# Shuijing725/CrowdNav_Prediction_AttnGraph

Hardware: NVIDIA H100
Metric: env_steps_per_s_ppo_rollout (higher is better)
Workload: dtype f32

## Files before the change

### crowdnav_prediction_attngraph_b200/csrc/cn_gemm_tc.cu

```cuda
#include "cn_gemm_tc.h"

__global__ void cn_split_f16_kernel(const float* __restrict__ src, float scale, __half* __restrict__ hi,
                                    __half* __restrict__ lo, size_t count) {
  const size_t i = (size_t)blockIdx.x * blockDim.x + threadIdx.x;
  if (i >= count) return;
  const float x = fminf(fmaxf(src[i] * scale, -65504.0f), 65504.0f);
  const __half h = __float2half_rn(x);
  hi[i] = h;
  lo[i] = __float2half_rn(x - __half2float(h));
}

namespace {

typedef CUresult (*EncodeFn)(CUtensorMap*, CUtensorMapDataType, cuuint32_t, void*, const cuuint64_t*, const cuuint64_t*,
                             const cuuint32_t*, const cuuint32_t*, CUtensorMapInterleave, CUtensorMapSwizzle,
                             CUtensorMapL2promotion, CUtensorMapFloatOOBfill);

EncodeFn get_encode() {
  static EncodeFn fn = nullptr;
  if (!fn) {
    void* sym = nullptr;
    cudaDriverEntryPointQueryResult qres;
    if (cudaGetDriverEntryPoint("cuTensorMapEncodeTiled", &sym, cudaEnableDefault, &qres) == cudaSuccess &&
        qres == cudaDriverEntryPointSuccess)
// ... 4 lines not shown

int halloc16(CnLaunchCtx* c, __half** ptr, size_t count) {
  float* q = nullptr;
  int rc = palloc(c, &q, (count + 1) / 2);
  *ptr = reinterpret_cast<__half*>(q);
  return rc;
}

int tc_store_maps(TcMat& t, int rows, int K) {
  if (!tma_store_ok(t.hi, (size_t)t.pitch * 2) || !tma_store_ok(t.lo, (size_t)t.pitch * 2)) return 0;
  int rc = make_store_map(&t.sh, t.hi, 2, rows, K, t.pitch);
  if (!rc) rc = make_store_map(&t.sl, t.lo, 2, rows, K, t.pitch);
  return rc;
}

typedef void (*TcKernel)(CUtensorMap, CUtensorMap, CUtensorMap, CUtensorMap, int, int, int, TcEpilogue, CUtensorMap,
                         CUtensorMap, CUtensorMap);
template <int BN>
TcKernel tc_kernel(int act, int out) {
  static const TcKernel k[3][3] = {
      {cn_gemm_tc_kernel<BN, false, CN_ACT_NONE, TC_OUT_F32>, cn_gemm_tc_kernel<BN, false, CN_ACT_NONE, TC_OUT_F16>,
       cn_gemm_tc_kernel<BN, false, CN_ACT_NONE, TC_OUT_BOTH>},
      {cn_gemm_tc_kernel<BN, false, CN_ACT_RELU, TC_OUT_F32>, cn_gemm_tc_kernel<BN, false, CN_ACT_RELU, TC_OUT_F16>,
       cn_gemm_tc_kernel<BN, false, CN_ACT_RELU, TC_OUT_BOTH>},
      {cn_gemm_tc_kernel<BN, false, CN_ACT_TANH, TC_OUT_F32>, cn_gemm_tc_kernel<BN, false, CN_ACT_TANH, TC_OUT_F16>,
       cn_gemm_tc_kernel<BN, false, CN_ACT_TANH, TC_OUT_BOTH>}};
  return k[act][out - 1];
}

#ifdef CN_GEMM_TRACE
unsigned long long* g_tc_trace = nullptr;
int g_tc_trace_cap = 0;
// ... 28 lines not shown
  CUresult r = enc(&s->map, esize == 4 ? CU_TENSOR_MAP_DATA_TYPE_FLOAT32 : CU_TENSOR_MAP_DATA_TYPE_FLOAT16, 2,
                   const_cast<void*>(ptr), gdim, gstride, box, estr, CU_TENSOR_MAP_INTERLEAVE_NONE,
                   CU_TENSOR_MAP_SWIZZLE_128B, CU_TENSOR_MAP_L2_PROMOTION_NONE, CU_TENSOR_MAP_FLOAT_OOB_FILL_NONE);
  if (r != CUDA_SUCCESS) return cn_set_error("cuTensorMapEncodeTiled(store) failed (%d) rows=%d cols=%d", (int)r, rows, cols);
  s->rows = rows; s->cols = cols;
  return 0;
}

int tc_alloc(CnLaunchCtx* c, TcMat& t, int rows, int K, int box_rows, int box_k) {
  int rc = halloc16(c, &t.hi, (size_t)rows * K);
  if (!rc) rc = halloc16(c, &t.lo, (size_t)rows * K);
  t.pitch = K; t.box_k = box_k;
  if (!rc) rc = make_map(&t.mh, t.hi, rows, K, box_rows, K, box_k);
  if (!rc) rc = make_map(&t.ml, t.lo, rows, K, box_rows, K, box_k);
  if (!rc) rc = tc_store_maps(t, rows, K);
  return rc;
}

int tc_view(TcMat& v, const TcMat& src, int col0, int rows, int K, int box_rows) {
  v.hi = src.hi + col0; v.lo = src.lo + col0; v.pitch = src.pitch; v.box_k = src.box_k;
  int rc = make_map(&v.mh, v.hi, rows, K, box_rows, src.pitch, src.box_k);
  if (!rc) rc = make_map(&v.ml, v.lo, rows, K, box_rows, src.pitch, src.box_k);
  if (!rc) rc = tc_store_maps(v, rows, K);
  return rc;
}

void split16(CnLaunchCtx* c, cudaStream_t st, const float* src, float scale, __half* hi, __half* lo, size_t count) {
  cn_split_f16_kernel<<<(unsigned)((count + 255) / 256), 256, 0, st>>>(src, scale, hi, lo, count);
  c->launches += 1;
}
// ... 5 lines not shown
      if (e == cudaSuccess)
        e = cudaFuncSetAttribute(tc_kernel<256>(act, out), cudaFuncAttributeMaxDynamicSharedMemorySize, TcCfg<256>::kSmemBytes);
      if (e == cudaSuccess)
        e = cudaFuncSetAttribute(tc_kernel<64>(act, out), cudaFuncAttributeMaxDynamicSharedMemorySize, TcCfg<64>::kSmemBytes);
    }
  if (e == cudaSuccess)
    e = cudaFuncSetAttribute(cn_gemm_tc_kernel<64, true>, cudaFuncAttributeMaxDynamicSharedMemorySize, TcCfg<64>::kSmemBytes);
  if (e == cudaSuccess)
    e = cudaFuncSetAttribute(cn_gemm_tc_kernel<256, false, CN_ACT_NONE, TC_OUT_GRU>,
                             cudaFuncAttributeMaxDynamicSharedMemorySize, TcCfg<256>::kSmemBytes);
  if (e != cudaSuccess) return cn_set_error("cudaFuncSetAttribute(tc): %s", cudaGetErrorString(e));
  return 0;
}

void gemm_tc(CnLaunchCtx* c, cudaStream_t st, const TcMat& A, const TcMat& B, int M, int N, int K, int bn, const float* bias,
             int act, const TcOut& o, const int* m_ptr, int act_lo, int act_hi, const int* m0_ptr) {
  TcEpilogue ep;
  memset(&ep, 0, sizeof(ep));
  ep.bias = bias; ep.inv_scale = 1.0f / 64.0f; ep.act = act; ep.act_lo = act_lo; ep.act_hi = act_hi;
  ep.c32 = o.c32; ep.ldc = o.ldc; ep.out_hi = o.oh; ep.out_lo = o.ol; ep.ldh = o.ldh; ep.m_ptr = m_ptr; ep.m0_ptr = m0_ptr;
  {
    static const int nostore = (getenv("CN_DBG_NOSTORE") && getenv("CN_DBG_NOSTORE")[0] == '1') ? 1 : 0;
    ep.dbg_nostore = nostore;
  }
  if (A.box_k != tc_box_k(bn) || B.box_k != tc_box_k(bn)) {
    if (!c->launch_error) {
      c->launch_error = true;
      cn_set_error("gemm_tc in stage '%s': operand boxes %d / %d wide, the BN = %d instance loads %d",
                   c->cur_stage ? c->cur_stage : "?", A.box_k, B.box_k, bn, tc_box_k(bn));
    }
    return;
  }
  const int out_kind = (o.c32 ? TC_OUT_F32 : 0) | (o.oh ? TC_OUT_F16 : 0);
  if (act < CN_ACT_NONE || act > CN_ACT_TANH || !out_kind) {
    if (!c->launch_error) {
      c->launch_error = true;
      cn_set_error("gemm_tc in stage '%s': activation %d / no output", c->cur_stage ? c->cur_stage : "?", act);
    }
    return;
  }
#ifdef CN_GEMM_TRACE
  ep.trace = g_tc_trace; ep.trace_cap = g_tc_trace_cap;
#endif
  static const CUtensorMap no_map = {};
// ... 3 lines not shown
    const bool ok = (!o.c32 || fits(o.sc)) && (!o.oh || (fits(o.sh) && fits(o.sl)));
    if (!ok) {
      if (!c->launch_error) {
        c->launch_error = true;
        cn_set_error("gemm_tc in stage '%s': a BN = 256 output needs a TMA store map of [%d x %d] (16-byte-aligned "
                     "base, row pitch a multiple of 16 bytes)", c->cur_stage ? c->cur_stage : "?", M, N);
      }
      return;
    }
    if (o.c32) mc = &o.sc->map;
    if (o.oh) { mh = &o.sh->map; ml = &o.sl->map; }
  }
  const int tiles = (N / bn) * ((M + TC_BM - 1) / TC_BM);
  dim3 grid(tiles < c->num_sms ? tiles : c->num_sms);
  if (bn == 256)
    launch_k(c, tc_kernel<256>(act, out_kind), grid, dim3(TC_THREADS), TcCfg<256>::kSmemBytes, st, A.mh, A.ml, B.mh, B.ml, M, N, K, ep,
             *mc, *mh, *ml);
  else
    launch_k(c, tc_kernel<64>(act, out_kind), grid, dim3(TC_THREADS), TcCfg<64>::kSmemBytes, st, A.mh, A.ml, B.mh, B.ml, M, N, K, ep,
             *mc, *mh, *ml);
}

void gemm_tc_gru(CnLaunchCtx* c, cudaStream_t st, const TcMat& A, const TcMat& B, int M, const float* bias,
                 const float* h_in, const float* mask, float* h_out, int group, int pitch, int off, __half* oh, __half* ol,
                 int ldh) {
  const int N = 4 * 256, K = 64 + 256;
  if (A.box_k != tc_box_k(256) || B.box_k != tc_box_k(256) || !bias || !h_out || !mask || group <= 0) {
    if (!c->launch_error) {
      c->launch_error = true;
      cn_set_error("gemm_tc_gru in stage '%s': operand boxes %d / %d wide (need %d), or a missing bias / mask / output",
                   c->cur_stage ? c->cur_stage : "?", A.box_k, B.box_k, tc_box_k(256));
    }
    return;
  }
  TcEpilogue ep;
  memset(&ep, 0, sizeof(ep));
  ep.bias = bias; ep.inv_scale = 1.0f / 64.0f; ep.act_hi = 1 << 30;
  ep.c32 = h_out; ep.ldc = 256; ep.out_hi = oh; ep.out_lo = ol; ep.ldh = ldh;
  ep.gru_h = h_in; ep.gru_mask = mask; ep.gru_group = group; ep.gru_pitch = pitch; ep.gru_off = off;
  static const CUtensorMap no_map = {};
  const int tiles = (N / 256) * ((M + TC_BM - 1) / TC_BM);
  dim3 grid(tiles < c->num_sms ? tiles : c->num_sms);
  launch_k(c, cn_gemm_tc_kernel<256, false, CN_ACT_NONE, TC_OUT_GRU>, grid, dim3(TC_THREADS), TcCfg<256>::kSmemBytes, st,
           A.mh, A.ml, B.mh, B.ml, M, N, K, ep, no_map, no_map, no_map);
}

int gemm_tc_promote(int num_sms, cudaStream_t st, const __half* ahi, const __half* alo, int a_rows, int a_pitch,
                    const __half* bhi, const __half* blo, int b_rows, int b_pitch, int Kd, float* C, int ldc,
                    const float* bias, int act, const float* inv_a, const float* inv_b, int ksplit) {
  const int bn = 64;
  if (b_rows % bn) return cn_set_error("cn_update gemm: output columns %d not a multiple of 64", b_rows);
  const int Kp = (Kd + TC_BK - 1) / TC_BK * TC_BK;
  CUtensorMap mah, mal, mbh, mbl;
  int rc = make_map(&mah, ahi, a_rows, Kd, TC_BM, a_pitch);
  if (!rc) rc = make_map(&mal, alo, a_rows, Kd, TC_BM, a_pitch);
  if (!rc) rc = make_map(&mbh, bhi, b_rows, Kd, bn, b_pitch);
  if (!rc) rc = make_map(&mbl, blo, b_rows, Kd, bn, b_pitch);
  if (rc) return rc;
  TcEpilogue ep;
  memset(&ep, 0, sizeof(ep));
  ep.bias = bias; ep.inv_scale = 1.0f; ep.act = act; ep.act_lo = 0; ep.act_hi = 1 << 30;
  ep.c32 = C; ep.ldc = ldc; ep.inv_scale_a = inv_a; ep.inv_scale_b = inv_b; ep.ksplit = ksplit;
  const int tiles = (b_rows / bn) * ((a_rows + TC_BM - 1) / TC_BM) * (ksplit > 1 ? ksplit : 1);
  const int grid = tiles < num_sms ? tiles : num_sms;
  static const CUtensorMap no_map = {};
  cn_gemm_tc_kernel<64, true><<<grid, TC_THREADS, TcCfg<64>::kSmemBytes, st>>>(mah, mal, mbh, mbl, a_rows, b_rows, Kp, ep,
                                                                                no_map, no_map, no_map);
  cudaError_t e = cudaGetLastError();
  if (e != cudaSuccess) return cn_set_error("cn_update gemm launch (M=%d N=%d K=%d ksplit=%d): %s", a_rows, b_rows, Kd, ksplit, cudaGetErrorString(e));
  return 0;
}

extern "C" {

int cn_internal_gemm_tc_ex(const float* dA, const float* dW, const float* dbias, float* dC, int M, int N, int K, int act,
                           int bn, const int* m_ptr, const int* m0_ptr, int a_col0, int a_pitch, __half* out_hi,
                           __half* out_lo, int ldh, int act_lo, int act_hi) {
  if (a_pitch == 0) a_pitch = K;
  if ((bn != 256 && bn != 64) || M <= 0 || N <= 0 || K <= 0 || N % bn || K % TC_BK || a_col0 < 0 ||
      a_col0 + K > a_pitch || a_col0 % 8 || a_pitch % 8 || (!dC && !out_hi) || (!out_hi != !out_lo) ||
      (out_hi && ldh < N))
    return cn_set_error("cn_internal_gemm_tc_ex: need bn in {64,256}, M, N, K > 0, N %% bn == 0, K %% 64 == 0, "
                        "a_col0 + K <= a_pitch (both multiples of 8), an output and ldh >= N");
  if (bn == 256 && ((dC && !tma_store_ok(dC, (size_t)N * 4)) ||
                    (out_hi && (!tma_store_ok(out_hi, (size_t)ldh * 2) || !tma_store_ok(out_lo, (size_t)ldh * 2)))))
    return cn_set_error("cn_internal_gemm_tc_ex: a BN = 256 output needs a 16-byte-aligned base and a row pitch that is "
                        "a multiple of 16 bytes");
  CnLaunchCtx ctx;
  cudaDeviceGetAttribute(&ctx.num_sms, cudaDevAttrMultiProcessorCount, 0);
  TcMat Af, A, B;
  int rc = tc_alloc(&ctx, Af, M, a_pitch, TC_BM, tc_box_k(bn));
  if (!rc) rc = tc_view(A, Af, a_col0, M, K, TC_BM);
  if (!rc) rc = tc_alloc(&ctx, B, N, K, bn, tc_box_k(bn));
  if (!rc) rc = tc_set_attrs();
  TcOut o = out32(dC, N);
  o.oh = out_hi; o.ol = out_lo; o.ldh = ldh;
  TcStoreMap sc, sh, sl;
  if (bn == 256) {
    if (!rc && dC) rc = make_store_map(&sc, dC, 4, M, N, N);
    if (!rc && out_hi) rc = make_store_map(&sh, out_hi, 2, M, N, ldh);
    if (!rc && out_hi) rc = make_store_map(&sl, out_lo, 2, M, N, ldh);
    o.sc = &sc; o.sh = &sh; o.sl = &sl;
  }
  if (!rc) {
    split16(&ctx, 0, dA, 1.0f, Af.hi, Af.lo, (size_t)M * a_pitch);
    split16(&ctx, 0, dW, 64.0f, B.hi, B.lo, (size_t)N * K);
    gemm_tc(&ctx, 0, A, B, M, N, K, bn, dbias, act, o, m_ptr, act_lo, act_hi > 0 ? act_hi : 1 << 30, m0_ptr);
    cudaError_t err = cudaDeviceSynchronize();
    if (err != cudaSuccess) rc = cn_set_error("cn_internal_gemm_tc_ex: %s", cudaGetErrorString(err));
    else if (ctx.launch_error) rc = 1;
  }
  cn_launch_free(&ctx);
  return rc;
}
int cn_internal_gemm_tc(const float* dA, const float* dW, const float* dbias, float* dC, int M, int N, int K, int act,
                        int bn) {
  return cn_internal_gemm_tc_ex(dA, dW, dbias, dC, M, N, K, act, bn, nullptr, nullptr, 0, 0, nullptr, nullptr, 0, 0, 0);
}

#ifdef CN_GEMM_TRACE
int cn_internal_gemm_trace(unsigned long long* dtrace, int cap) {
  g_tc_trace = dtrace; g_tc_trace_cap = dtrace ? cap : 0;
  return 0;
}
#endif

}
```

### crowdnav_prediction_attngraph_b200/csrc/cn_gemm_tc.cuh

```cuda
#pragma once
#include <cuda.h>
#include <cuda_fp16.h>
#include <cuda_runtime.h>
#include <stdint.h>

#include "cn_launch.cuh"

#define TC_BM 128
#define TC_BK 64
#define TC_CONSUMER_WARPS 8
#define TC_THREADS (128 + 32 * TC_CONSUMER_WARPS)

template <int BN>
struct TcCfg {
  static constexpr int kBK = (BN >= 256) ? 32 : TC_BK;
  static constexpr int kSwizzle = 2 * kBK;
  static constexpr int kStages = 4;
  static constexpr int kATile = TC_BM * kBK * 2;
  static constexpr int kBTile = BN * kBK * 2;
  static constexpr int kStageBytes = 2 * kATile + 2 * kBTile;
  static constexpr int kStoreBoxes = (BN >= 256) ? 2 : 0;
  static constexpr int kBoxBytes = 64 * 128;
  static constexpr int kStagingBytes = 2 * kStoreBoxes * kBoxBytes;
  static constexpr int kSmemBytes = kStages * kStageBytes + kStagingBytes + 256  + 1024 ;
};

struct TcEpilogue {
  const float* bias;
  float inv_scale;
  int act;
  int act_lo, act_hi;
  float* c32;
  int ldc;
  __half* out_hi;
  __half* out_lo;
  int ldh;
  const int* m_ptr;
  int dbg_nostore;
  const int* m0_ptr;
  const float* inv_scale_a;
  const float* inv_scale_b;
  int ksplit;
  const float* gru_h;
  const float* gru_mask;
  int gru_group, gru_pitch, gru_off;
#ifdef CN_GEMM_TRACE
  unsigned long long* trace;
  int trace_cap;
#endif
};

#ifdef CN_GEMM_TRACE
#define TC_TRACE_REC 7
#define TC_TRACE_WAIT_CLK 100
#endif

enum { TC_OUT_F32 = 1, TC_OUT_F16 = 2, TC_OUT_BOTH = 3, TC_OUT_GRU = 4 };

#ifdef CN_GEMM_TRACE
#define TC_TRACE(...) __VA_ARGS__
#else
#define TC_TRACE(...)
#endif

namespace tc {

__device__ __forceinline__ uint32_t smem_u32(const void* p) { return (uint32_t)__cvta_generic_to_shared(p); }

// ... 82 lines not shown

template <int N>
__device__ __forceinline__ void wgmma_f16(float (&d)[N / 2], uint64_t da, uint64_t db, uint32_t accum);
template <>
__device__ __forceinline__ void wgmma_f16<64>(float (&d)[32], uint64_t da, uint64_t db, uint32_t accum) {
  asm volatile(
      "{\n.reg .pred p;\nsetp.ne.b32 p, %34, 0;\n"
      "wgmma.mma_async.sync.aligned.m64n64k16.f32.f16.f16 {"
      "%0, %1, %2, %3, %4, %5, %6, %7, %8, %9, %10, %11, %12, %13, %14, %15, "
      "%16, %17, %18, %19, %20, %21, %22, %23, %24, %25, %26, %27, %28, %29, %30, %31"
      "}, %32, %33, p, 1, 1, 0, 0;\n}\n"
      : "+f"(d[0]), "+f"(d[1]), "+f"(d[2]), "+f"(d[3]), "+f"(d[4]), "+f"(d[5]), "+f"(d[6]), "+f"(d[7]),
        "+f"(d[8]), "+f"(d[9]), "+f"(d[10]), "+f"(d[11]), "+f"(d[12]), "+f"(d[13]), "+f"(d[14]), "+f"(d[15]),
        "+f"(d[16]), "+f"(d[17]), "+f"(d[18]), "+f"(d[19]), "+f"(d[20]), "+f"(d[21]), "+f"(d[22]), "+f"(d[23]),
        "+f"(d[24]), "+f"(d[25]), "+f"(d[26]), "+f"(d[27]), "+f"(d[28]), "+f"(d[29]), "+f"(d[30]), "+f"(d[31])
      : "l"(da), "l"(db), "r"(accum));
}
template <>
__device__ __forceinline__ void wgmma_f16<192>(float (&d)[96], uint64_t da, uint64_t db, uint32_t accum) {
  asm volatile(
      "{\n.reg .pred p;\nsetp.ne.b32 p, %98, 0;\n"
      "wgmma.mma_async.sync.aligned.m64n192k16.f32.f16.f16 {"
      "%0, %1, %2, %3, %4, %5, %6, %7, %8, %9, %10, %11, %12, %13, %14, %15, "
      "%16, %17, %18, %19, %20, %21, %22, %23, %24, %25, %26, %27, %28, %29, %30, %31, "
      "%32, %33, %34, %35, %36, %37, %38, %39, %40, %41, %42, %43, %44, %45, %46, %47, "
      "%48, %49, %50, %51, %52, %53, %54, %55, %56, %57, %58, %59, %60, %61, %62, %63, "
      "%64, %65, %66, %67, %68, %69, %70, %71, %72, %73, %74, %75, %76, %77, %78, %79, "
      "%80, %81, %82, %83, %84, %85, %86, %87, %88, %89, %90, %91, %92, %93, %94, %95"
      "}, %96, %97, p, 1, 1, 0, 0;\n}\n"
      : "+f"(d[0]), "+f"(d[1]), "+f"(d[2]), "+f"(d[3]), "+f"(d[4]), "+f"(d[5]), "+f"(d[6]), "+f"(d[7]),
// ... 114 lines not shown
#else
      tc::bulk_wait_read<PENDING>();
#endif
    }
    tc::named_bar_sync(bar_id, 128);
  }
  __device__ __forceinline__ void release() {
    tc::fence_proxy_async_smem();
    tc::named_bar_sync(bar_id, 128);
  }
  __device__ __forceinline__ uint32_t buf(uint32_t b) const { return base + (b % TcCfg<256>::kStoreBoxes) * TcCfg<256>::kBoxBytes; }
};

template <int ACT, int OUT>
__device__ __forceinline__ void tc_epilogue_tma(const float (&acc)[128], const TcEpilogue& ep, float inv_scale, int n0,
                                                int m_half, int wr, int lane, TcStaging& sg, const CUtensorMap* map_c,
                                                const CUtensorMap* map_oh, const CUtensorMap* map_ol) {
  static_assert(ACT >= 0 && ACT <= 2 && OUT >= TC_OUT_F32 && OUT <= TC_OUT_BOTH, "epilogue kind");
  constexpr int NB = TcCfg<256>::kStoreBoxes;
  static_assert(NB >= 2 && (NB & (NB - 1)) == 0, "the split fp16 output stages hi and lo boxes together");
  const int cq = 2 * (lane & 3);
  const bool issue = sg.leader && !ep.dbg_nostore;
  const uint32_t rsw = (uint32_t)(wr & 7);
  const uint32_t row_off = (uint32_t)wr * 128u;
  if constexpr ((OUT & TC_OUT_F32) != 0) {
#pragma unroll
    for (int j = 0; j < 8; ++j) {
      sg.acquire<NB - 1>();
      const uint32_t b = sg.buf(sg.box) + row_off + 8u * (uint32_t)(lane & 1);
#pragma unroll
      for (int q = 0; q < 4; ++q) {
        const int g = 4 * j + q, col = n0 + 8 * g + cq;
        const float b0 = ep.bias ? __ldg(ep.bias + col) : 0.0f, b1 = ep.bias ? __ldg(ep.bias + col + 1) : 0.0f;
        const bool w0 = col >= ep.act_lo && col < ep.act_hi, w1 = col + 1 >= ep.act_lo && col + 1 < ep.act_hi;
        const uint32_t chunk = (uint32_t)(2 * q + ((lane & 3) >> 1));
#pragma unroll
        for (int h = 0; h < 2; ++h) {
          float v0 = fmaf(acc[4 * g + 2 * h], inv_scale, b0), v1 = fmaf(acc[4 * g + 2 * h + 1], inv_scale, b1);
          if constexpr (ACT == 1) {
            v0 = w0 ? fmaxf(v0, 0.0f) : v0; v1 = w1 ? fmaxf(v1, 0.0f) : v1;
          } else if constexpr (ACT == 2) {
            if (w0) v0 = tc::fast_tanh(v0);
// ... 1 lines not shown
          }
          tc::st_shared_v2(b + 1024u * h + ((chunk ^ rsw) << 4), v0, v1);
        }
      }
      sg.release();
      if (issue) {
        tc::tma_store_2d(map_c, sg.buf(sg.box), n0 + 32 * j, m_half);
        tc::bulk_commit();
      }
      ++sg.box;
    }
  }
  if constexpr ((OUT & TC_OUT_F16) != 0) {
#pragma unroll
    for (int j = 0; j < 4; ++j) {
      sg.acquire<NB - 2>();
      const uint32_t bh = sg.buf(sg.box) + row_off + 4u * (uint32_t)(lane & 3);
      const uint32_t bl = sg.buf(sg.box + 1) + row_off + 4u * (uint32_t)(lane & 3);
#pragma unroll
      for (int q = 0; q < 8; ++q) {
        const int g = 8 * j + q, col = n0 + 8 * g + cq;
        const float b0 = ep.bias ? __ldg(ep.bias + col) : 0.0f, b1 = ep.bias ? __ldg(ep.bias + col + 1) : 0.0f;
        const bool w0 = col >= ep.act_lo && col < ep.act_hi, w1 = col + 1 >= ep.act_lo && col + 1 < ep.act_hi;
        const uint32_t sw_off = ((uint32_t)q ^ rsw) << 4;
#pragma unroll
        for (int h = 0; h < 2; ++h) {
          float v0 = fmaf(acc[4 * g + 2 * h], inv_scale, b0), v1 = fmaf(acc[4 * g + 2 * h + 1], inv_scale, b1);
          if constexpr (ACT == 1) {
            v0 = w0 ? fmaxf(v0, 0.0f) : v0; v1 = w1 ? fmaxf(v1, 0.0f) : v1;
          } else if constexpr (ACT == 2) {
// ... 49 lines not shown
        o[k] = (1.0f - z) * n + z * hv[k];
      }
      if (ep.dbg_nostore) continue;
      *reinterpret_cast<float2*>(ep.c32 + orow * 256 + u) = make_float2(o[0], o[1]);
      if (ep.out_hi) {
        uint32_t lo;
        const uint32_t hi = tc::split_pair_hi(o[0], o[1], &lo);
        const size_t q = (size_t)row * ep.ldh + u;
        *reinterpret_cast<uint32_t*>(ep.out_hi + q) = hi;
        *reinterpret_cast<uint32_t*>(ep.out_lo + q) = lo;
      }
    }
  }
}

template <int BN, bool PROMOTE = false, int ACT = 0, int OUT = TC_OUT_F32>
__global__ void __launch_bounds__(TC_THREADS, 1)
cn_gemm_tc_kernel(const __grid_constant__ CUtensorMap map_ahi, const __grid_constant__ CUtensorMap map_alo,
                  const __grid_constant__ CUtensorMap map_bhi, const __grid_constant__ CUtensorMap map_blo,
                  int M, int N, int K, TcEpilogue ep, const __grid_constant__ CUtensorMap map_c,
                  const __grid_constant__ CUtensorMap map_oh, const __grid_constant__ CUtensorMap map_ol) {
  cn_pdl_trigger();
  constexpr int TC_STAGES = TcCfg<BN>::kStages;
  constexpr int BK = TcCfg<BN>::kBK;
  constexpr int SW = TcCfg<BN>::kSwizzle;
  constexpr int TC_A_TILE_BYTES = TcCfg<BN>::kATile;
  constexpr int TC_B_TILE_BYTES = TcCfg<BN>::kBTile;
  constexpr int TC_STAGE_BYTES = TcCfg<BN>::kStageBytes;
  constexpr bool kTmaStore = !PROMOTE && BN == 256 && OUT != TC_OUT_GRU;
  static_assert(OUT != TC_OUT_GRU || (BN == 256 && !PROMOTE), "the GRU epilogue reads four 64-column gate blocks");
  static_assert(!PROMOTE || BK == 64, "PROMOTE sums 64-wide k-blocks");
  static_assert(!kTmaStore || TcCfg<BN>::kStoreBoxes > 0, "BN = 256 stages its output");
  extern __shared__ uint8_t tc_smem_raw[];
  const uint32_t raw = tc::smem_u32(tc_smem_raw);
  const uint32_t base = (raw + 1023u) & ~1023u;
  const uint32_t staging = base + TC_STAGES * TC_STAGE_BYTES;
  const uint32_t bar_base = staging + TcCfg<BN>::kStagingBytes;
  const uint32_t bar_full = bar_base, bar_empty = bar_base + 64;

  const int warp = threadIdx.x >> 5, lane = threadIdx.x & 31, wg = warp >> 2;
  const int num_kb = K / BK;

  if (threadIdx.x == 0) {
    for (int s = 0; s < TC_STAGES; ++s) {
      tc::mbar_init(bar_full + 8 * s, 1);
      tc::mbar_init(bar_empty + 8 * s, TC_CONSUMER_WARPS);
    }
    asm volatile("fence.mbarrier_init.release.cluster;" ::: "memory");
    asm volatile("prefetch.tensormap [%0];" ::"l"(&map_ahi) : "memory");
    asm volatile("prefetch.tensormap [%0];" ::"l"(&map_alo) : "memory");
    asm volatile("prefetch.tensormap [%0];" ::"l"(&map_bhi) : "memory");
    asm volatile("prefetch.tensormap [%0];" ::"l"(&map_blo) : "memory");
    if constexpr (kTmaStore) {
      if constexpr ((OUT & TC_OUT_F32) != 0) asm volatile("prefetch.tensormap [%0];" ::"l"(&map_c) : "memory");
      if constexpr ((OUT & TC_OUT_F16) != 0) {
        asm volatile("prefetch.tensormap [%0];" ::"l"(&map_oh) : "memory");
        asm volatile("prefetch.tensormap [%0];" ::"l"(&map_ol) : "memory");
      }
    }
  }
  __syncthreads();
  cn_pdl_wait();
  const int m_ext = M;
  if (ep.m_ptr) { const int mc = *ep.m_ptr; M = mc < M ? mc : M; }
  int m_lo = ep.m0_ptr ? *ep.m0_ptr : 0;
  if (m_lo > M) m_lo = M;
  const int n_ntiles = N / BN;
  const int n_mn = ((M - m_lo + TC_BM - 1) / TC_BM) * n_ntiles;
  const int ksplit = (PROMOTE && ep.ksplit > 1) ? ep.ksplit : 1;
  const int kb_per = (num_kb + ksplit - 1) / ksplit;
  const int n_tiles = n_mn * ksplit;

  if (wg == 0) {
    tc::setmaxnreg_dec<40>();
    if (threadIdx.x == 0) {
      uint32_t it = 0;
      for (int tile = blockIdx.x; tile < n_tiles; tile += gridDim.x) {
        const int mn = tile % n_mn, ks = tile / n_mn;
        const int m0 = m_lo + (mn / n_ntiles) * TC_BM, n0 = (mn % n_ntiles) * BN;
        const int kb0 = ks * kb_per, kb1 = (kb0 + kb_per < num_kb) ? kb0 + kb_per : num_kb;
        for (int kb = kb0; kb < kb1; ++kb, ++it) {
          const uint32_t s = it % TC_STAGES, ph = (it / TC_STAGES) & 1u;
          tc::mbar_wait(bar_empty + 8 * s, ph ^ 1u);
          const uint32_t full = bar_full + 8 * s;
          tc::mbar_expect_tx(full, TC_STAGE_BYTES);
          const uint32_t st = base + s * TC_STAGE_BYTES;
          tc::tma_load_2d(st, &map_ahi, full, kb * BK, m0);
          tc::tma_load_2d(st + TC_A_TILE_BYTES, &map_alo, full, kb * BK, m0);
          tc::tma_load_2d(st + 2 * TC_A_TILE_BYTES, &map_bhi, full, kb * BK, n0);
          tc::tma_load_2d(st + 2 * TC_A_TILE_BYTES + TC_B_TILE_BYTES, &map_blo, full, kb * BK, n0);
        }
      }
    }
    return;
  }
  tc::setmaxnreg_inc<232>();
  float inv_scale = ep.inv_scale;
  if (ep.inv_scale_a) inv_scale *= __ldg(ep.inv_scale_a);
  if (ep.inv_scale_b) inv_scale *= __ldg(ep.inv_scale_b);
  const int half = wg - 1;
  const int wr = 16 * (warp & 3) + (lane >> 2);
  const int cq = 2 * (lane & 3);
  uint32_t it = 0;
  TcStaging sg;
  sg.base = staging + half * TcCfg<BN>::kStoreBoxes * TcCfg<BN>::kBoxBytes;
  sg.box = 0; sg.leader = (threadIdx.x & 127) == 0; sg.bar_id = wg;
  TC_TRACE(sg.waits = 0; sg.wait_clk = 0;)
  TC_TRACE(const bool tr = ep.trace && warp == 4 && lane == 0; int tr_n = 0;)
  for (int tile = blockIdx.x; tile < n_tiles; tile += gridDim.x) {
    const int mn = tile % n_mn, ks = tile / n_mn;
    const int m0 = m_lo + (mn / n_ntiles) * TC_BM, n0 = (mn % n_ntiles) * BN;
    const int kb0 = ks * kb_per, kb1 = (kb0 + kb_per < num_kb) ? kb0 + kb_per : num_kb;
    TC_TRACE(const uint64_t t_tile = tc::globaltimer(); uint64_t t_first = 0; uint32_t polls = 0;)
    float acc[BN / 2];
    float sum[PROMOTE ? BN / 2 : 1];
    if constexpr (PROMOTE) {
#pragma unroll
      for (int i = 0; i < BN / 2; ++i) sum[i] = 0.0f;
    }
    uint32_t prev = 0;
    for (int kb = kb0; kb < kb1; ++kb, ++it) {
      const uint32_t s = it % TC_STAGES, ph = (it / TC_STAGES) & 1u;
#ifdef CN_GEMM_TRACE
      polls += tc::mbar_wait_polls(bar_full + 8 * s, ph);
      if (kb == kb0) t_first = tc::globaltimer();
#else
      tc::mbar_wait(bar_full + 8 * s, ph);
#endif
      const uint32_t st = base + s * TC_STAGE_BYTES;
      const uint32_t a_hi = st + half * (TC_A_TILE_BYTES / 2), a_lo = a_hi + TC_A_TILE_BYTES,
                     b_hi = st + 2 * TC_A_TILE_BYTES, b_lo = b_hi + TC_B_TILE_BYTES;
      tc::fence_regs(acc);
      tc::wgmma_fence();
#pragma unroll
      for (int k = 0; k < BK / 16; ++k) {
        const uint32_t koff = k * 32;
        const uint64_t dah = tc::make_desc<SW>(a_hi + koff), dal = tc::make_desc<SW>(a_lo + koff);
        const uint64_t dbh = tc::make_desc<SW>(b_hi + koff), dbl = tc::make_desc<SW>(b_lo + koff);
        const bool first = k == 0 && (PROMOTE || kb == kb0);
        tc::wgmma_f16<BN>(acc, dah, dbh, first ? 0u : 1u);
        tc::wgmma_f16<BN>(acc, dah, dbl, 1u);
        tc::wgmma_f16<BN>(acc, dal, dbh, 1u);
      }
      tc::wgmma_commit();
      tc::fence_regs(acc);
      if constexpr (PROMOTE) {
        tc::wgmma_wait<0>();
        tc::fence_regs(acc);
        __syncwarp();
        if (lane == 0) tc::mbar_arrive(bar_empty + 8 * s);
#pragma unroll
        for (int i = 0; i < BN / 2; ++i) sum[i] += acc[i];
      } else {
        tc::wgmma_wait<1>();
        if (kb != kb0) {
          __syncwarp();
          if (lane == 0) tc::mbar_arrive(bar_empty + 8 * prev);
        }
        prev = s;
// ... 3 lines not shown
#pragma unroll
      for (int i = 0; i < BN / 2; ++i) acc[i] = sum[i];
    } else {
      tc::wgmma_wait<0>();
      tc::fence_regs(acc);
      __syncwarp();
      if (lane == 0) tc::mbar_arrive(bar_empty + 8 * prev);
    }

    TC_TRACE(const uint64_t t_loop = tc::globaltimer();)
    if constexpr (!PROMOTE) {
      TC_TRACE(const uint32_t waits0 = sg.waits; const uint64_t clk0 = sg.wait_clk;)
      if constexpr (OUT == TC_OUT_GRU) {
        tc_epilogue_gru(acc, ep, inv_scale, n0, m0 + 64 * half + wr, cq, m_ext);
      } else if constexpr (kTmaStore) {
        tc_epilogue_tma<ACT, OUT>(acc, ep, inv_scale, n0, m0 + 64 * half, wr, lane, sg, &map_c, &map_oh, &map_ol);
      } else {
        tc_epilogue_store<BN, ACT, OUT>(acc, ep, inv_scale, n0, m0 + 64 * half + wr, cq, m_ext);
      }
      TC_TRACE(
        if (tr && tr_n < ep.trace_cap) {
          unsigned long long* rec = ep.trace + ((size_t)blockIdx.x * ep.trace_cap + tr_n) * TC_TRACE_REC;
          rec[0] = t_tile; rec[1] = t_first; rec[2] = t_loop; rec[3] = tc::globaltimer(); rec[4] = polls;
          rec[5] = sg.waits - waits0; rec[6] = sg.wait_clk - clk0;
        }
        ++tr_n;)
      continue;
    }
    const bool act_full = ep.act_lo <= n0 && ep.act_hi >= n0 + BN;
    const bool act_none = ep.act == 0 || ep.act_hi <= n0 || ep.act_lo >= n0 + BN;
    const int act_mode = act_none ? 0 : (act_full ? ep.act : 3);
    const bool with_bias = ep.bias && ks == 0;
    const int r0 = m0 + 64 * half + wr;
#pragma unroll
    for (int g = 0; g < BN / 8; ++g) {
      const int col = n0 + 8 * g + cq;
      const float b0 = with_bias ? __ldg(ep.bias + col) : 0.0f, b1 = with_bias ? __ldg(ep.bias + col + 1) : 0.0f;
#pragma unroll
      for (int h = 0; h < 2; ++h) {
// ... 35 lines not shown
```

### crowdnav_prediction_attngraph_b200/csrc/cn_gemm_tc.h

```cpp
#pragma once
#include <cuda.h>
#include <cuda_fp16.h>
#include <cuda_runtime.h>
#include <stdint.h>

#include "cn_gemm_tc.cuh"
#include "cn_launch.cuh"

struct TcStoreMap {
  CUtensorMap map;
  int rows = 0, cols = 0;
};

struct TcMat {
  __half *hi = nullptr, *lo = nullptr;
  CUtensorMap mh, ml;
  int pitch = 0;
  int box_k = 0;
  TcStoreMap sh, sl;
};

struct TcOut {
  float* c32 = nullptr; int ldc = 0;
  __half *oh = nullptr, *ol = nullptr; int ldh = 0;
  const TcStoreMap *sc = nullptr, *sh = nullptr, *sl = nullptr;
};
inline TcOut out32(float* c, int ldc, const TcStoreMap* sc = nullptr) { TcOut o; o.c32 = c; o.ldc = ldc; o.sc = sc; return o; }
inline TcOut out16(const TcMat& t) { TcOut o; o.oh = t.hi; o.ol = t.lo; o.ldh = t.pitch; o.sh = &t.sh; o.sl = &t.sl; return o; }
inline TcOut out_both(float* c, int ldc, const TcMat& t) { TcOut o = out16(t); o.c32 = c; o.ldc = ldc; return o; }

inline int tc_box_k(int bn) { return bn == 256 ? TcCfg<256>::kBK : TcCfg<64>::kBK; }

inline bool tma_store_ok(const void* ptr, size_t pitch_bytes) { return ((uintptr_t)ptr % 16) == 0 && pitch_bytes % 16 == 0; }

int make_map(CUtensorMap* map, const __half* ptr, int rows, int K, int box_rows, int pitch, int box_k = TC_BK);
int make_store_map(TcStoreMap* s, const void* ptr, int esize, int rows, int cols, int pitch);
int tc_alloc(CnLaunchCtx* c, TcMat& t, int rows, int K, int box_rows, int box_k);
int tc_view(TcMat& v, const TcMat& src, int col0, int rows, int K, int box_rows);
void split16(CnLaunchCtx* c, cudaStream_t st, const float* src, float scale, __half* hi, __half* lo, size_t count);
int tc_set_attrs();

void gemm_tc(CnLaunchCtx* c, cudaStream_t st, const TcMat& A, const TcMat& B, int M, int N, int K, int bn, const float* bias,
             int act, const TcOut& o, const int* m_ptr = nullptr, int act_lo = 0, int act_hi = 1 << 30,
             const int* m0_ptr = nullptr);

void gemm_tc_gru(CnLaunchCtx* c, cudaStream_t st, const TcMat& A, const TcMat& B, int M, const float* bias,
                 const float* h_in, const float* mask, float* h_out, int group, int pitch, int off, __half* oh, __half* ol,
                 int ldh);

int gemm_tc_promote(int num_sms, cudaStream_t st, const __half* ahi, const __half* alo, int a_rows, int a_pitch,
                    const __half* bhi, const __half* blo, int b_rows, int b_pitch, int Kd, float* C, int ldc,
                    const float* bias, int act, const float* inv_a, const float* inv_b, int ksplit);
```

Before: 6.793 million.

## Split tail-wave GEMM tiles into narrower N sub-tiles to balance the last wave

Adds a persistent-kernel schedule that, for the remainder tiles beyond the last full wave, splits each BN=256 tile into up to four narrower N sub-tiles (64 or 128 wide) so more SMs share the tail work. Sub-tile B operands are loaded through extra TMA maps with smaller boxes, and narrower wgmma instances are used. The epilogue stores only the active width. This adds two tensormap parameters, branchy MMA dispatch and extra A-tile reloads for split tiles, in exchange for reduced tail-wave imbalance.

```diff
diff --git a/crowdnav_prediction_attngraph_b200/csrc/cn_gemm_tc.cu b/crowdnav_prediction_attngraph_b200/csrc/cn_gemm_tc.cu
--- a/crowdnav_prediction_attngraph_b200/csrc/cn_gemm_tc.cu
+++ b/crowdnav_prediction_attngraph_b200/csrc/cn_gemm_tc.cu
@@ -42,8 +42,8 @@
   return rc;
 }
 
-typedef void (*TcKernel)(CUtensorMap, CUtensorMap, CUtensorMap, CUtensorMap, int, int, int, TcEpilogue, CUtensorMap,
-                         CUtensorMap, CUtensorMap);
+typedef void (*TcKernel)(CUtensorMap, CUtensorMap, CUtensorMap, CUtensorMap, CUtensorMap, CUtensorMap, int, int, int,
+                         TcEpilogue, CUtensorMap, CUtensorMap, CUtensorMap);
 template <int BN>
 TcKernel tc_kernel(int act, int out) {
   static const TcKernel k[3][3] = {
@@ -102,6 +102,12 @@
   if (!rc) rc = make_map(&t.mh, t.hi, rows, K, box_rows, K, box_k);
   if (!rc) rc = make_map(&t.ml, t.lo, rows, K, box_rows, K, box_k);
   if (!rc) rc = tc_store_maps(t, rows, K);
+  if (!rc && box_rows == 256 && box_k == tc_box_k(256)) {
+    const int sub = TcCfg<256>::kSubN;
+    rc = make_map(&t.msh, t.hi, rows, K, sub, K, box_k);
+    if (!rc) rc = make_map(&t.msl, t.lo, rows, K, sub, K, box_k);
+    if (!rc) t.sub_rows = sub;
+  }
   return rc;
 }
 
@@ -137,20 +143,22 @@
 }
 
 void gemm_tc(CnLaunchCtx* c, cudaStream_t st, const TcMat& A, const TcMat& B, int M, int N, int K, int bn, const float* bias,
-             int act, const TcOut& o, const int* m_ptr, int act_lo, int act_hi, const int* m0_ptr) {
+             int act, const TcOut& o, const int* m_ptr, int act_lo, int act_hi, const int* m0_ptr, int max_split) {
   TcEpilogue ep;
   memset(&ep, 0, sizeof(ep));
   ep.bias = bias; ep.inv_scale = 1.0f / 64.0f; ep.act = act; ep.act_lo = act_lo; ep.act_hi = act_hi;
   ep.c32 = o.c32; ep.ldc = o.ldc; ep.out_hi = o.oh; ep.out_lo = o.ol; ep.ldh = o.ldh; ep.m_ptr = m_ptr; ep.m0_ptr = m0_ptr;
+  ep.max_split = max_split;
   {
     static const int nostore = (getenv("CN_DBG_NOSTORE") && getenv("CN_DBG_NOSTORE")[0] == '1') ? 1 : 0;
     ep.dbg_nostore = nostore;
   }
-  if (A.box_k != tc_box_k(bn) || B.box_k != tc_box_k(bn)) {
+  if (A.box_k != tc_box_k(bn) || B.box_k != tc_box_k(bn) || (bn == 256 && B.sub_rows != TcCfg<256>::kSubN)) {
     if (!c->launch_error) {
       c->launch_error = true;
-      cn_set_error("gemm_tc in stage '%s': operand boxes %d / %d wide, the BN = %d instance loads %d",
-                   c->cur_stage ? c->cur_stage : "?", A.box_k, B.box_k, bn, tc_box_k(bn));
+      cn_set_error("gemm_tc in stage '%s': operand boxes %d / %d wide and B sub-tile boxes of %d rows, the BN = %d "
+                   "instance loads %d (and sub-tile boxes of %d rows for BN = 256)", c->cur_stage ? c->cur_stage : "?",
+                   A.box_k, B.box_k, B.sub_rows, bn, tc_box_k(bn), TcCfg<256>::kSubN);
     }
     return;
   }
@@ -184,11 +192,11 @@
   const int tiles = (N / bn) * ((M + TC_BM - 1) / TC_BM);
   dim3 grid(tiles < c->num_sms ? tiles : c->num_sms);
   if (bn == 256)
-    launch_k(c, tc_kernel<256>(act, out_kind), grid, dim3(TC_THREADS), TcCfg<256>::kSmemBytes, st, A.mh, A.ml, B.mh, B.ml, M, N, K, ep,
-             *mc, *mh, *ml);
+    launch_k(c, tc_kernel<256>(act, out_kind), grid, dim3(TC_THREADS), TcCfg<256>::kSmemBytes, st, A.mh, A.ml, B.mh, B.ml,
+             B.msh, B.msl, M, N, K, ep, *mc, *mh, *ml);
   else
-    launch_k(c, tc_kernel<64>(act, out_kind), grid, dim3(TC_THREADS), TcCfg<64>::kSmemBytes, st, A.mh, A.ml, B.mh, B.ml, M, N, K, ep,
-             *mc, *mh, *ml);
+    launch_k(c, tc_kernel<64>(act, out_kind), grid, dim3(TC_THREADS), TcCfg<64>::kSmemBytes, st, A.mh, A.ml, B.mh, B.ml,
+             B.msh, B.msl, M, N, K, ep, *mc, *mh, *ml);
 }
 
 void gemm_tc_gru(CnLaunchCtx* c, cudaStream_t st, const TcMat& A, const TcMat& B, int M, const float* bias,
@@ -212,7 +220,7 @@
   const int tiles = (N / 256) * ((M + TC_BM - 1) / TC_BM);
   dim3 grid(tiles < c->num_sms ? tiles : c->num_sms);
   launch_k(c, cn_gemm_tc_kernel<256, false, CN_ACT_NONE, TC_OUT_GRU>, grid, dim3(TC_THREADS), TcCfg<256>::kSmemBytes, st,
-           A.mh, A.ml, B.mh, B.ml, M, N, K, ep, no_map, no_map, no_map);
+           A.mh, A.ml, B.mh, B.ml, no_map, no_map, M, N, K, ep, no_map, no_map, no_map);
 }
 
 int gemm_tc_promote(int num_sms, cudaStream_t st, const __half* ahi, const __half* alo, int a_rows, int a_pitch,
@@ -234,8 +242,8 @@
   const int tiles = (b_rows / bn) * ((a_rows + TC_BM - 1) / TC_BM) * (ksplit > 1 ? ksplit : 1);
   const int grid = tiles < num_sms ? tiles : num_sms;
   static const CUtensorMap no_map = {};
-  cn_gemm_tc_kernel<64, true><<<grid, TC_THREADS, TcCfg<64>::kSmemBytes, st>>>(mah, mal, mbh, mbl, a_rows, b_rows, Kp, ep,
-                                                                                no_map, no_map, no_map);
+  cn_gemm_tc_kernel<64, true><<<grid, TC_THREADS, TcCfg<64>::kSmemBytes, st>>>(mah, mal, mbh, mbl, no_map, no_map, a_rows,
+                                                                                b_rows, Kp, ep, no_map, no_map, no_map);
   cudaError_t e = cudaGetLastError();
   if (e != cudaSuccess) return cn_set_error("cn_update gemm launch (M=%d N=%d K=%d ksplit=%d): %s", a_rows, b_rows, Kd, ksplit, cudaGetErrorString(e));
   return 0;
@@ -243,9 +251,9 @@
 
 extern "C" {
 
-int cn_internal_gemm_tc_ex(const float* dA, const float* dW, const float* dbias, float* dC, int M, int N, int K, int act,
-                           int bn, const int* m_ptr, const int* m0_ptr, int a_col0, int a_pitch, __half* out_hi,
-                           __half* out_lo, int ldh, int act_lo, int act_hi) {
+int cn_internal_gemm_tc_split(const float* dA, const float* dW, const float* dbias, float* dC, int M, int N, int K, int act,
+                              int bn, const int* m_ptr, const int* m0_ptr, int a_col0, int a_pitch, __half* out_hi,
+                              __half* out_lo, int ldh, int act_lo, int act_hi, int max_split) {
   if (a_pitch == 0) a_pitch = K;
   if ((bn != 256 && bn != 64) || M <= 0 || N <= 0 || K <= 0 || N % bn || K % TC_BK || a_col0 < 0 ||
       a_col0 + K > a_pitch || a_col0 % 8 || a_pitch % 8 || (!dC && !out_hi) || (!out_hi != !out_lo) ||
@@ -275,7 +283,7 @@
   if (!rc) {
     split16(&ctx, 0, dA, 1.0f, Af.hi, Af.lo, (size_t)M * a_pitch);
     split16(&ctx, 0, dW, 64.0f, B.hi, B.lo, (size_t)N * K);
-    gemm_tc(&ctx, 0, A, B, M, N, K, bn, dbias, act, o, m_ptr, act_lo, act_hi > 0 ? act_hi : 1 << 30, m0_ptr);
+    gemm_tc(&ctx, 0, A, B, M, N, K, bn, dbias, act, o, m_ptr, act_lo, act_hi > 0 ? act_hi : 1 << 30, m0_ptr, max_split);
     cudaError_t err = cudaDeviceSynchronize();
     if (err != cudaSuccess) rc = cn_set_error("cn_internal_gemm_tc_ex: %s", cudaGetErrorString(err));
     else if (ctx.launch_error) rc = 1;
@@ -283,6 +291,15 @@
   cn_launch_free(&ctx);
   return rc;
 }
+int cn_internal_gemm_tc_ex(const float* dA, const float* dW, const float* dbias, float* dC, int M, int N, int K, int act,
+                           int bn, const int* m_ptr, const int* m0_ptr, int a_col0, int a_pitch, __half* out_hi,
+                           __half* out_lo, int ldh, int act_lo, int act_hi) {
+  return cn_internal_gemm_tc_split(dA, dW, dbias, dC, M, N, K, act, bn, m_ptr, m0_ptr, a_col0, a_pitch, out_hi, out_lo, ldh,
+                                   act_lo, act_hi, 0);
+}
+int cn_internal_gemm_tc_tail_split(int tiles, int grid, int bn, int max_split) {
+  return tc_schedule(tiles, grid, tc_split_cap(bn == 256 ? TcCfg<256>::kMaxSplit : TcCfg<64>::kMaxSplit, max_split)).split;
+}
 int cn_internal_gemm_tc(const float* dA, const float* dW, const float* dbias, float* dC, int M, int N, int K, int act,
                         int bn) {
   return cn_internal_gemm_tc_ex(dA, dW, dbias, dC, M, N, K, act, bn, nullptr, nullptr, 0, 0, nullptr, nullptr, 0, 0, 0);
diff --git a/crowdnav_prediction_attngraph_b200/csrc/cn_gemm_tc.cuh b/crowdnav_prediction_attngraph_b200/csrc/cn_gemm_tc.cuh
--- a/crowdnav_prediction_attngraph_b200/csrc/cn_gemm_tc.cuh
+++ b/crowdnav_prediction_attngraph_b200/csrc/cn_gemm_tc.cuh
@@ -23,7 +23,32 @@
   static constexpr int kBoxBytes = 64 * 128;
   static constexpr int kStagingBytes = 2 * kStoreBoxes * kBoxBytes;
   static constexpr int kSmemBytes = kStages * kStageBytes + kStagingBytes + 256  + 1024 ;
+  static constexpr int kMaxSplit = (BN >= 256) ? 4 : 1;
+  static constexpr int kSubN = BN / kMaxSplit;
 };
+
+struct TcSched {
+  int whole;
+  int split;
+  int total;
+};
+__host__ __device__ inline TcSched tc_schedule(int tiles, int grid, int max_split) {
+  const int whole = tiles / grid * grid, r = tiles - whole;
+  int s = 1;
+  for (int c = 2; c <= max_split; c *= 2)
+    if (((c * r + grid - 1) / grid) * s < ((s * r + grid - 1) / grid) * c) s = c;
+  return {whole, s, whole + s * r};
+}
+__host__ __device__ inline int tc_split_cap(int cap, int asked) { return (asked > 0 && asked < cap) ? asked : cap; }
+struct TcItem {
+  int tile, col, width;
+};
+template <int BN>
+__device__ __forceinline__ TcItem tc_item(int t, const TcSched& sc) {
+  if (t < sc.whole) return {t, 0, BN};
+  const int u = t - sc.whole, w = BN / sc.split;
+  return {sc.whole + u / sc.split, (u % sc.split) * w, w};
+}
 
 struct TcEpilogue {
   const float* bias;
@@ -38,6 +63,7 @@
   const int* m_ptr;
   int dbg_nostore;
   const int* m0_ptr;
+  int max_split;
   const float* inv_scale_a;
   const float* inv_scale_b;
   int ksplit;
@@ -51,7 +77,7 @@
 };
 
 #ifdef CN_GEMM_TRACE
-#define TC_TRACE_REC 7
+#define TC_TRACE_REC 8
 #define TC_TRACE_WAIT_CLK 100
 #endif
 
@@ -164,6 +190,26 @@
         "+f"(d[8]), "+f"(d[9]), "+f"(d[10]), "+f"(d[11]), "+f"(d[12]), "+f"(d[13]), "+f"(d[14]), "+f"(d[15]),
         "+f"(d[16]), "+f"(d[17]), "+f"(d[18]), "+f"(d[19]), "+f"(d[20]), "+f"(d[21]), "+f"(d[22]), "+f"(d[23]),
         "+f"(d[24]), "+f"(d[25]), "+f"(d[26]), "+f"(d[27]), "+f"(d[28]), "+f"(d[29]), "+f"(d[30]), "+f"(d[31])
+      : "l"(da), "l"(db), "r"(accum));
+}
+template <>
+__device__ __forceinline__ void wgmma_f16<128>(float (&d)[64], uint64_t da, uint64_t db, uint32_t accum) {
+  asm volatile(
+      "{\n.reg .pred p;\nsetp.ne.b32 p, %66, 0;\n"
+      "wgmma.mma_async.sync.aligned.m64n128k16.f32.f16.f16 {"
+      "%0, %1, %2, %3, %4, %5, %6, %7, %8, %9, %10, %11, %12, %13, %14, %15, "
+      "%16, %17, %18, %19, %20, %21, %22, %23, %24, %25, %26, %27, %28, %29, %30, %31, "
+      "%32, %33, %34, %35, %36, %37, %38, %39, %40, %41, %42, %43, %44, %45, %46, %47, "
+      "%48, %49, %50, %51, %52, %53, %54, %55, %56, %57, %58, %59, %60, %61, %62, %63"
+      "}, %64, %65, p, 1, 1, 0, 0;\n}\n"
+      : "+f"(d[0]), "+f"(d[1]), "+f"(d[2]), "+f"(d[3]), "+f"(d[4]), "+f"(d[5]), "+f"(d[6]), "+f"(d[7]),
+        "+f"(d[8]), "+f"(d[9]), "+f"(d[10]), "+f"(d[11]), "+f"(d[12]), "+f"(d[13]), "+f"(d[14]), "+f"(d[15]),
+        "+f"(d[16]), "+f"(d[17]), "+f"(d[18]), "+f"(d[19]), "+f"(d[20]), "+f"(d[21]), "+f"(d[22]), "+f"(d[23]),
+        "+f"(d[24]), "+f"(d[25]), "+f"(d[26]), "+f"(d[27]), "+f"(d[28]), "+f"(d[29]), "+f"(d[30]), "+f"(d[31]),
+        "+f"(d[32]), "+f"(d[33]), "+f"(d[34]), "+f"(d[35]), "+f"(d[36]), "+f"(d[37]), "+f"(d[38]), "+f"(d[39]),
+        "+f"(d[40]), "+f"(d[41]), "+f"(d[42]), "+f"(d[43]), "+f"(d[44]), "+f"(d[45]), "+f"(d[46]), "+f"(d[47]),
+        "+f"(d[48]), "+f"(d[49]), "+f"(d[50]), "+f"(d[51]), "+f"(d[52]), "+f"(d[53]), "+f"(d[54]), "+f"(d[55]),
+        "+f"(d[56]), "+f"(d[57]), "+f"(d[58]), "+f"(d[59]), "+f"(d[60]), "+f"(d[61]), "+f"(d[62]), "+f"(d[63])
       : "l"(da), "l"(db), "r"(accum));
 }
 template <>
@@ -308,8 +354,9 @@
 
 template <int ACT, int OUT>
 __device__ __forceinline__ void tc_epilogue_tma(const float (&acc)[128], const TcEpilogue& ep, float inv_scale, int n0,
-                                                int m_half, int wr, int lane, TcStaging& sg, const CUtensorMap* map_c,
-                                                const CUtensorMap* map_oh, const CUtensorMap* map_ol) {
+                                                int width, int m_half, int wr, int lane, TcStaging& sg,
+                                                const CUtensorMap* map_c, const CUtensorMap* map_oh,
+                                                const CUtensorMap* map_ol) {
   static_assert(ACT >= 0 && ACT <= 2 && OUT >= TC_OUT_F32 && OUT <= TC_OUT_BOTH, "epilogue kind");
   constexpr int NB = TcCfg<256>::kStoreBoxes;
   static_assert(NB >= 2 && (NB & (NB - 1)) == 0, "the split fp16 output stages hi and lo boxes together");
@@ -320,6 +367,7 @@
   if constexpr ((OUT & TC_OUT_F32) != 0) {
 #pragma unroll
     for (int j = 0; j < 8; ++j) {
+      if (32 * j >= width) break;
       sg.acquire<NB - 1>();
       const uint32_t b = sg.buf(sg.box) + row_off + 8u * (uint32_t)(lane & 1);
 #pragma unroll
@@ -351,6 +399,7 @@
   if constexpr ((OUT & TC_OUT_F16) != 0) {
 #pragma unroll
     for (int j = 0; j < 4; ++j) {
+      if (64 * j >= width) break;
       sg.acquire<NB - 2>();
       const uint32_t bh = sg.buf(sg.box) + row_off + 4u * (uint32_t)(lane & 3);
       const uint32_t bl = sg.buf(sg.box + 1) + row_off + 4u * (uint32_t)(lane & 3);
@@ -430,10 +479,45 @@
   }
 }
 
+template <int W, int BN, int SW, int BK>
+__device__ __forceinline__ void tc_mma_kblock(float (&acc)[BN / 2], uint32_t a_hi, uint32_t a_lo, uint32_t b_hi,
+                                              uint32_t b_lo, bool start) {
+  float (&d)[W / 2] = *reinterpret_cast<float (*)[W / 2]>(&acc[0]);
+  tc::wgmma_fence();
+#pragma unroll
+  for (int k = 0; k < BK / 16; ++k) {
+    const uint32_t koff = k * 32;
+    const uint64_t dah = tc::make_desc<SW>(a_hi + koff), dal = tc::make_desc<SW>(a_lo + koff);
+    const uint64_t dbh = tc::make_desc<SW>(b_hi + koff), dbl = tc::make_desc<SW>(b_lo + koff);
+    tc::wgmma_f16<W>(d, dah, dbh, (start && k == 0) ? 0u : 1u);
+    tc::wgmma_f16<W>(d, dah, dbl, 1u);
+    tc::wgmma_f16<W>(d, dal, dbh, 1u);
+  }
+  tc::wgmma_commit();
+}
+template <int BN, int SW, int BK, bool TAIL>
+__device__ __forceinline__ void tc_mma_kblock_w(float (&acc)[BN / 2], int width, uint32_t a_hi, uint32_t a_lo,
+                                                uint32_t b_hi, uint32_t b_lo, bool start) {
+  if constexpr (TAIL) {
+    if (width == TcCfg<BN>::kSubN) {
+      tc_mma_kblock<TcCfg<BN>::kSubN, BN, SW, BK>(acc, a_hi, a_lo, b_hi, b_lo, start);
+      return;
+    }
+    if constexpr (TcCfg<BN>::kMaxSplit >= 4) {
+      if (width == BN / 2) {
+        tc_mma_kblock<BN / 2, BN, SW, BK>(acc, a_hi, a_lo, b_hi, b_lo, start);
+        return;
+      }
+    }
+  }
+  tc_mma_kblock<BN, BN, SW, BK>(acc, a_hi, a_lo, b_hi, b_lo, start);
+}
+
 template <int BN, bool PROMOTE = false, int ACT = 0, int OUT = TC_OUT_F32>
 __global__ void __launch_bounds__(TC_THREADS, 1)
 cn_gemm_tc_kernel(const __grid_constant__ CUtensorMap map_ahi, const __grid_constant__ CUtensorMap map_alo,
                   const __grid_constant__ CUtensorMap map_bhi, const __grid_constant__ CUtensorMap map_blo,
+                  const __grid_constant__ CUtensorMap map_bshi, const __grid_constant__ CUtensorMap map_bslo,
                   int M, int N, int K, TcEpilogue ep, const __grid_constant__ CUtensorMap map_c,
                   const __grid_constant__ CUtensorMap map_oh, const __grid_constant__ CUtensorMap map_ol) {
   cn_pdl_trigger();
@@ -444,6 +528,9 @@
   constexpr int TC_B_TILE_BYTES = TcCfg<BN>::kBTile;
   constexpr int TC_STAGE_BYTES = TcCfg<BN>::kStageBytes;
   constexpr bool kTmaStore = !PROMOTE && BN == 256 && OUT != TC_OUT_GRU;
+  constexpr bool kTail = !PROMOTE && OUT != TC_OUT_GRU && TcCfg<BN>::kMaxSplit > 1;
+  constexpr int kSubN = TcCfg<BN>::kSubN;
+  static_assert(!kTmaStore || kSubN % 64 == 0, "a sub-tile stores whole 64-column boxes");
   static_assert(OUT != TC_OUT_GRU || (BN == 256 && !PROMOTE), "the GRU epilogue reads four 64-column gate blocks");
   static_assert(!PROMOTE || BK == 64, "PROMOTE sums 64-wide k-blocks");
   static_assert(!kTmaStore || TcCfg<BN>::kStoreBoxes > 0, "BN = 256 stages its output");
@@ -467,6 +554,10 @@
     asm volatile("prefetch.tensormap [%0];" ::"l"(&map_alo) : "memory");
     asm volatile("prefetch.tensormap [%0];" ::"l"(&map_bhi) : "memory");
     asm volatile("prefetch.tensormap [%0];" ::"l"(&map_blo) : "memory");
+    if constexpr (kTail) {
+      asm volatile("prefetch.tensormap [%0];" ::"l"(&map_bshi) : "memory");
+      asm volatile("prefetch.tensormap [%0];" ::"l"(&map_bslo) : "memory");
+    }
     if constexpr (kTmaStore) {
       if constexpr ((OUT & TC_OUT_F32) != 0) asm volatile("prefetch.tensormap [%0];" ::"l"(&map_c) : "memory");
       if constexpr ((OUT & TC_OUT_F16) != 0) {
@@ -486,25 +577,35 @@
   const int ksplit = (PROMOTE && ep.ksplit > 1) ? ep.ksplit : 1;
   const int kb_per = (num_kb + ksplit - 1) / ksplit;
   const int n_tiles = n_mn * ksplit;
+  const TcSched sched = tc_schedule(n_tiles, gridDim.x, kTail ? tc_split_cap(TcCfg<BN>::kMaxSplit, ep.max_split) : 1);
 
   if (wg == 0) {
     tc::setmaxnreg_dec<40>();
     if (threadIdx.x == 0) {
       uint32_t it = 0;
-      for (int tile = blockIdx.x; tile < n_tiles; tile += gridDim.x) {
-        const int mn = tile % n_mn, ks = tile / n_mn;
-        const int m0 = m_lo + (mn / n_ntiles) * TC_BM, n0 = (mn % n_ntiles) * BN;
+      for (int t = blockIdx.x; t < sched.total; t += gridDim.x) {
+        const TcItem wi = tc_item<BN>(t, sched);
+        const int mn = wi.tile % n_mn, ks = wi.tile / n_mn;
+        const int m0 = m_lo + (mn / n_ntiles) * TC_BM, n0 = (mn % n_ntiles) * BN + wi.col;
         const int kb0 = ks * kb_per, kb1 = (kb0 + kb_per < num_kb) ? kb0 + kb_per : num_kb;
         for (int kb = kb0; kb < kb1; ++kb, ++it) {
           const uint32_t s = it % TC_STAGES, ph = (it / TC_STAGES) & 1u;
           tc::mbar_wait(bar_empty + 8 * s, ph ^ 1u);
           const uint32_t full = bar_full + 8 * s;
-          tc::mbar_expect_tx(full, TC_STAGE_BYTES);
+          tc::mbar_expect_tx(full, 2 * TC_A_TILE_BYTES + 2 * wi.width * BK * 2);
           const uint32_t st = base + s * TC_STAGE_BYTES;
           tc::tma_load_2d(st, &map_ahi, full, kb * BK, m0);
           tc::tma_load_2d(st + TC_A_TILE_BYTES, &map_alo, full, kb * BK, m0);
-          tc::tma_load_2d(st + 2 * TC_A_TILE_BYTES, &map_bhi, full, kb * BK, n0);
-          tc::tma_load_2d(st + 2 * TC_A_TILE_BYTES + TC_B_TILE_BYTES, &map_blo, full, kb * BK, n0);
+          if (wi.width == BN) {
+            tc::tma_load_2d(st + 2 * TC_A_TILE_BYTES, &map_bhi, full, kb * BK, n0);
+            tc::tma_load_2d(st + 2 * TC_A_TILE_BYTES + TC_B_TILE_BYTES, &map_blo, full, kb * BK, n0);
+          } else {
+            for (int j = 0; j < wi.width; j += kSubN) {
+              const uint32_t off = 2 * TC_A_TILE_BYTES + j * BK * 2;
+              tc::tma_load_2d(st + off, &map_bshi, full, kb * BK, n0 + j);
+              tc::tma_load_2d(st + off + TC_B_TILE_BYTES, &map_bslo, full, kb * BK, n0 + j);
+            }
+          }
         }
       }
     }
@@ -523,9 +624,10 @@
   sg.box = 0; sg.leader = (threadIdx.x & 127) == 0; sg.bar_id = wg;
   TC_TRACE(sg.waits = 0; sg.wait_clk = 0;)
   TC_TRACE(const bool tr = ep.trace && warp == 4 && lane == 0; int tr_n = 0;)
-  for (int tile = blockIdx.x; tile < n_tiles; tile += gridDim.x) {
-    const int mn = tile % n_mn, ks = tile / n_mn;
-    const int m0 = m_lo + (mn / n_ntiles) * TC_BM, n0 = (mn % n_ntiles) * BN;
+  for (int t = blockIdx.x; t < sched.total; t += gridDim.x) {
+    const TcItem wi = tc_item<BN>(t, sched);
+    const int mn = wi.tile % n_mn, ks = wi.tile / n_mn;
+    const int m0 = m_lo + (mn / n_ntiles) * TC_BM, n0 = (mn % n_ntiles) * BN + wi.col;
     const int kb0 = ks * kb_per, kb1 = (kb0 + kb_per < num_kb) ? kb0 + kb_per : num_kb;
     TC_TRACE(const uint64_t t_tile = tc::globaltimer(); uint64_t t_first = 0; uint32_t polls = 0;)
     float acc[BN / 2];
@@ -547,18 +649,7 @@
       const uint32_t a_hi = st + half * (TC_A_TILE_BYTES / 2), a_lo = a_hi + TC_A_TILE_BYTES,
                      b_hi = st + 2 * TC_A_TILE_BYTES, b_lo = b_hi + TC_B_TILE_BYTES;
       tc::fence_regs(acc);
-      tc::wgmma_fence();
-#pragma unroll
-      for (int k = 0; k < BK / 16; ++k) {
-        const uint32_t koff = k * 32;
-        const uint64_t dah = tc::make_desc<SW>(a_hi + koff), dal = tc::make_desc<SW>(a_lo + koff);
-        const uint64_t dbh = tc::make_desc<SW>(b_hi + koff), dbl = tc::make_desc<SW>(b_lo + koff);
-        const bool first = k == 0 && (PROMOTE || kb == kb0);
-        tc::wgmma_f16<BN>(acc, dah, dbh, first ? 0u : 1u);
-        tc::wgmma_f16<BN>(acc, dah, dbl, 1u);
-        tc::wgmma_f16<BN>(acc, dal, dbh, 1u);
-      }
-      tc::wgmma_commit();
+      tc_mma_kblock_w<BN, SW, BK, kTail>(acc, wi.width, a_hi, a_lo, b_hi, b_lo, PROMOTE || kb == kb0);
       tc::fence_regs(acc);
       if constexpr (PROMOTE) {
         tc::wgmma_wait<0>();
@@ -592,7 +683,8 @@
       if constexpr (OUT == TC_OUT_GRU) {
         tc_epilogue_gru(acc, ep, inv_scale, n0, m0 + 64 * half + wr, cq, m_ext);
       } else if constexpr (kTmaStore) {
-        tc_epilogue_tma<ACT, OUT>(acc, ep, inv_scale, n0, m0 + 64 * half, wr, lane, sg, &map_c, &map_oh, &map_ol);
+        tc_epilogue_tma<ACT, OUT>(acc, ep, inv_scale, n0, wi.width, m0 + 64 * half, wr, lane, sg, &map_c, &map_oh,
+                                  &map_ol);
       } else {
         tc_epilogue_store<BN, ACT, OUT>(acc, ep, inv_scale, n0, m0 + 64 * half + wr, cq, m_ext);
       }
@@ -600,7 +692,7 @@
         if (tr && tr_n < ep.trace_cap) {
           unsigned long long* rec = ep.trace + ((size_t)blockIdx.x * ep.trace_cap + tr_n) * TC_TRACE_REC;
           rec[0] = t_tile; rec[1] = t_first; rec[2] = t_loop; rec[3] = tc::globaltimer(); rec[4] = polls;
-          rec[5] = sg.waits - waits0; rec[6] = sg.wait_clk - clk0;
+          rec[5] = sg.waits - waits0; rec[6] = sg.wait_clk - clk0; rec[7] = (unsigned long long)wi.width;
         }
         ++tr_n;)
       continue;
diff --git a/crowdnav_prediction_attngraph_b200/csrc/cn_gemm_tc.h b/crowdnav_prediction_attngraph_b200/csrc/cn_gemm_tc.h
--- a/crowdnav_prediction_attngraph_b200/csrc/cn_gemm_tc.h
+++ b/crowdnav_prediction_attngraph_b200/csrc/cn_gemm_tc.h
@@ -18,6 +18,8 @@
   int pitch = 0;
   int box_k = 0;
   TcStoreMap sh, sl;
+  CUtensorMap msh, msl;
+  int sub_rows = 0;
 };
 
 struct TcOut {
@@ -42,7 +44,7 @@
 
 void gemm_tc(CnLaunchCtx* c, cudaStream_t st, const TcMat& A, const TcMat& B, int M, int N, int K, int bn, const float* bias,
              int act, const TcOut& o, const int* m_ptr = nullptr, int act_lo = 0, int act_hi = 1 << 30,
-             const int* m0_ptr = nullptr);
+             const int* m0_ptr = nullptr, int max_split = 0);
 
 void gemm_tc_gru(CnLaunchCtx* c, cudaStream_t st, const TcMat& A, const TcMat& B, int M, const float* bias,
                  const float* h_in, const float* mask, float* h_out, int group, int pitch, int off, __half* oh, __half* ol,
```

Measured after the change: 6.763 million, median of 6. No clear change (-0.4%).
